# facebookresearch/Pearl

Hardware: NVIDIA H100
Metric: learner gradient-steps/sec (batch=256, 1e6 replay) (higher is better)
Workload: dtype f32 (3xTF32 tensor-core products, fp32 accumulate)

## Files before the change

### pearl_b200/csrc/dqn_common.cuh

```cuda
#pragma once
#include "common.cuh"
#include "host_runtime.cuh"

namespace prl {

struct Dims {
    int obs, A, H1, H2, D, H1p, H2p, P, Pp;
    int oW1, ob1, oW2, ob2, oW3, ob3;
};

__host__ __device__ inline Dims make_dims(int obs, int A, int H1, int H2) {
    Dims d;
    d.obs = obs; d.A = A; d.H1 = H1; d.H2 = H2; d.D = obs + A;
    d.H1p = round_up(H1, 4); d.H2p = round_up(H2, 4);
    d.oW1 = 0; d.ob1 = d.oW1 + H1 * d.D; d.oW2 = d.ob1 + H1; d.ob2 = d.oW2 + H2 * H1;
    d.oW3 = d.ob2 + H2; d.ob3 = d.oW3 + H2; d.P = d.ob3 + 1;
    d.Pp = round_up(d.P + 1, 4);
    return d;
}


__device__ __forceinline__ float soft_update(float src, float tgt, float tau, float omtau) {
    return __fadd_rn(__fmul_rn(tau, src), __fmul_rn(omtau, tgt));
}


struct AdamScalars {
    float decay, omb1, beta2, omb2, eps, step_size, bc2_sqrt;
};
__device__ __forceinline__ float adamw_step(float *w, float *m_, float *v_, float *vmax_, float g, const AdamScalars &h) {
    float p = __fmul_rn(__ldcg(w), h.decay);
    float m = __ldcg(m_);
    m = fmaf(h.omb1, g - m, m);
    float v = __fmul_rn(__ldcg(v_), h.beta2);
    v = __fadd_rn(v, __fmul_rn(__fmul_rn(h.omb2, g), g));
    const float vm = fmaxf(__ldcg(vmax_), v);
    const float denom = __fadd_rn(__fdiv_rn(__fsqrt_rn(vm), h.bc2_sqrt), h.eps);
    p = __fadd_rn(p, __fdiv_rn(__fmul_rn(-h.step_size, m), denom));
    *w = p; *m_ = m; *v_ = v; *vmax_ = vm;
    return p;
}

}

struct prl_dqn {
    prl_dqn_cfg cfg;
    prl::Dims d;
    float *w, *wt, *m, *v, *vmax;
    int64_t adam_step;
    float *gpart;
    int32_t *slots, *logical;
    float2 *scal_dev;
    uint32_t *tmp_rec;
    float *is_w, *td;
    void *multi_dev;
    float *tc_tiles;
    int32_t *tmp_slots;
    prl_buf_layout tmp_lay;
    prl::Stage stage;
    int sm_count, max_smem;
    int learn_smem, qv_smem;
    int last_launches, last_ctas, last_rows;
    int timing;
    cudaEvent_t t0, t1;
    long long *prof;
    prl_comm *comm;
};


int prl_dqn_stage_scalars(prl_dqn *q, int rounds, cudaStream_t stream);

inline int64_t prl_tc_tile_floats(const prl_dqn_cfg *c) {
    if (c->hidden1 != 64 || c->hidden2 != 64 || c->obs_dim > 128 || c->obs_dim % 8) return 0;
    return 2ll * (128 * ((c->obs_dim + 63) & ~63) + 2 * 64 * 64);
}
```

### pearl_b200/csrc/dqn_tc.cu

```cuda
#include <math.h>
#include <stdarg.h>
#include <stdlib.h>

#include <new>

#include "dqn_common.cuh"
#include "sampler.cuh"
#include "umma.cuh"

using namespace prl;

int prl_sampler_params(const prl_buf *b, int k, prl::SamplerParams *sp, size_t *smem_bytes);

namespace {

constexpr int NTH = 256;
constexpr int HID = 64;
constexpr int MAX_B = 256;
constexpr int REG1 = 0, REG2 = 65536, REG3 = 131072, MISC_OFF = 196608;
constexpr int HALF = 32768;
constexpr int SBUF = 16384;
constexpr int TL = 144;
constexpr int AR_A_HI = 0, AR_A_LO = 18432, AR_B_HI = 36864, AR_B_LO = 73728, AR_E = 110592;
constexpr int ACH = 1024, ARING = 8, ASLOT = 4 * ACH * 4;

struct TcLearner {
    const uint32_t *records;
    float *tiles;
    const int32_t *slots;
    float *w, *wt, *m, *v, *vmax;
    const float2 *scal;
    float *out_mae, *out_q, *out_y;
    long long steps0;
    int buf_flags;
    int pad_;
};

struct TcArgs {
    const TcLearner *learners;
    prl_buf_layout lay;
    Dims d;
    int B, rounds, freq;
    int round0;
    float decay, omb1, beta2, omb2, eps, gamma, tau, omtau, inv_b2;
    long long *prof;
    int prof_cta;
    int adam_tma;
};

#define TC_STAMP(idx)                                                                          \
    do {                                                                                       \
        if (a.prof && blockIdx.x == a.prof_cta && threadIdx.x == 0) a.prof[(size_t)round * 16 + (idx)] = clock64(); \
    } while (0)

struct Misc {
    struct Smalls { float watb[16][HID]; float b2[HID], w3[HID]; float b3, pad0[3]; } sm[2];
    float y[MAX_B];
    int act[MAX_B], cnt[MAX_B], slot[MAX_B];
    float rew[MAX_B], term[MAX_B];
    float redw[8][HID];
    float redmae[8], reddb3[8];
    unsigned long long bar[3 + ARING];
    TcLearner L;
    float dw3[16][NTH];
};

__device__ __forceinline__ void cp_async16_zfill_tc(void *smem_dst, const void *gmem_src, int src_bytes) {
    unsigned sa = (unsigned)__cvta_generic_to_shared(smem_dst);
    asm volatile("cp.async.cg.shared.global [%0], [%1], 16, %2;\n" ::"r"(sa), "l"(gmem_src), "r"(src_bytes) : "memory");
}

__device__ __forceinline__ int tid_here() {
    int t = threadIdx.x;
    asm volatile("" : "+r"(t));
    return t;
}
__device__ __forceinline__ int acc_row_here(int p) {
    const int t = tid_here();
    return ((t >> 5) & 3) * 16 + ((t & 31) >> 2) + 8 * p;
}
__device__ __forceinline__ void group_sync(int g) { asm volatile("bar.sync %0, %1;" ::"r"(1 + g), "r"(128) : "memory"); }

__device__ __forceinline__ void mbar_expect_tx(uint64_t *bar, uint32_t bytes) {
    asm volatile("mbarrier.arrive.expect_tx.shared::cta.b64 _, [%0], %1;" ::"r"(umma::smem_u32(bar)), "r"(bytes) : "memory");
}
__device__ __forceinline__ void bulk_g2s(void *smem_dst, const void *gmem_src, uint32_t bytes, uint64_t *bar) {
    asm volatile("cp.async.bulk.shared::cluster.global.mbarrier::complete_tx::bytes [%0], [%1], %2, [%3];"
                 ::"r"(umma::smem_u32(smem_dst)), "l"(gmem_src), "r"(bytes), "r"(umma::smem_u32(bar))
                 : "memory");
}
__device__ __forceinline__ void fence_proxy_async_all() { asm volatile("fence.proxy.async;" ::: "memory"); }
using umma::tf32_lo;

struct NetTiles { float *w1hi, *w1lo, *w2; };
__host__ __device__ inline int k1_cols(int obs) { return (obs + 63) & ~63; }
__host__ __device__ inline int net_tile_floats(int obs) { return 128 * k1_cols(obs) + 2 * HID * HID; }
__device__ __forceinline__ NetTiles net_tiles(float *base, int obs) {
    const int k1 = k1_cols(obs);
    return NetTiles{base, base + 64 * k1, base + 128 * k1};
}
__device__ void rebuild_tiles(const float *__restrict__ net, const Dims &d, const NetTiles &t, int tid) {
    const int k1 = k1_cols(d.obs);
    for (int e = tid; e < HID * k1; e += NTH) {
        const int j = e / k1, k = e - j * k1;
        const float x = k < d.obs ? __ldcg(net + d.oW1 + (size_t)j * d.D + k) : 0.f;
        const int idx = umma::tile_index(j, k, k1);
        t.w1hi[idx] = x; t.w1lo[idx] = tf32_lo(x);
    }
    for (int e = tid; e < HID * HID; e += NTH) {
        const int j = e >> 6, k = e & 63;
        const float x = __ldcg(net + d.oW2 + e);
        const int i1 = umma::tile_index(j, umma::kperm(k), HID);
        t.w2[i1] = x; t.w2[4096 + i1] = tf32_lo(x);
    }
}
__device__ void load_smalls(const float *__restrict__ net, const Dims &d, Misc::Smalls &mi) {
    const int tid = tid_here();
    float wa[4], bb[4];
#pragma unroll
    for (int u = 0; u < 4; u++) {
        const int e = tid + u * NTH;
        if (e < d.A * HID) {
            const int j = e / d.A, a = e - j * d.A;
            wa[u] = __ldcg(net + d.oW1 + (size_t)j * d.D + d.obs + a);
            bb[u] = __ldcg(net + d.ob1 + j);
        }
    }
#pragma unroll
    for (int u = 0; u < 4; u++) {
        const int e = tid + u * NTH;
        if (e < d.A * HID) { const int j = e / d.A, a = e - j * d.A; mi.watb[a][j] = wa[u] + bb[u]; }
    }
    if (tid < HID) { mi.b2[tid] = __ldcg(net + d.ob2 + tid); mi.w3[tid] = __ldcg(net + d.oW3 + tid); }
    if (tid == 0) mi.b3 = __ldcg(net + d.ob3);
}

__device__ __forceinline__ float fast_sqrt(float x) {
    float r;
    asm("sqrt.approx.f32 %0, %1;" : "=f"(r) : "f"(x));
    return r;
}
struct AdamScalarsTc : AdamScalars { float inv_bc2_sqrt; };

__device__ __forceinline__ float adam_math(float w, float &m, float &v, float &x, float g, const AdamScalarsTc &hs) {
    float p = __fmul_rn(w, hs.decay);
    m = fmaf(hs.omb1, g - m, m);
    v = __fadd_rn(__fmul_rn(v, hs.beta2), __fmul_rn(__fmul_rn(hs.omb2, g), g));
    x = fmaxf(x, v);
    const float denom = __fadd_rn(__fmul_rn(fast_sqrt(x), hs.inv_bc2_sqrt), hs.eps);
    return __fadd_rn(p, __fdividef(__fmul_rn(-hs.step_size, m), denom));
}

__device__ __forceinline__ void l1_issue(const TcArgs &a, const TcLearner &L, const Misc &mi, char *smem, int field_off, int row0, int kc) {
    const int ft = tid_here(), m = ft & 127, g = ft >> 7;
    float *sbuf = reinterpret_cast<float *>(smem + REG2 + g * 2 * SBUF + (kc & 1) * SBUF);
#pragma unroll 4
    for (int i = 0; i < 8; i++) {
        const int item = i * 128 + m, rr = item >> 4, c = item & 15, k = kc * 64 + c * 4;
        const float *src = reinterpret_cast<const float *>(L.records + (size_t)mi.slot[row0 + rr] * a.lay.record_words) + field_off + k;
        const int nb = k < a.d.obs ? 16 : 0;
        cp_async16_zfill_tc(sbuf + rr * 64 + ((c ^ (rr & 7)) << 2), nb ? src : reinterpret_cast<const float *>(L.records), nb);
    }
    cp_async_commit();
}
__device__ __forceinline__ void layer1_block(const TcArgs &a, const TcLearner &L, const Misc &mi, char *smem, int field_off, int row0,
                                             float (&t1)[32]) {
// ... 33 lines not shown
            for (int e = 0; e < 2; e++) umma::split_tf32(v[4 * j + 2 * p + e], hi[4 * j + 2 * e + p], lo[4 * j + 2 * e + p]);
}

__device__ __forceinline__ float2 lds2(const float *p) {
    float2 v;
    asm volatile("ld.shared.v2.f32 {%0, %1}, [%2];" : "=f"(v.x), "=f"(v.y) : "r"(umma::smem_u32(p)));
    return v;
}

__device__ __forceinline__ float warp_sum(float v) {
#pragma unroll
    for (int o = 16; o; o >>= 1) v += __shfl_xor_sync(0xffffffffu, v, o);
    return v;
}
__device__ __forceinline__ float quad_sum(float v) {
    v += __shfl_xor_sync(0xffffffffu, v, 1);
    return v + __shfl_xor_sync(0xffffffffu, v, 2);
}

__host__ __device__ inline int dw1_share(int obs) { return obs > 64 ? 64 : obs > 32 ? 32 : obs > 16 ? 16 : 8; }

__device__ const uint8_t kIota[16] = {0, 1, 2, 3, 4, 5, 6, 7, 8, 9, 10, 11, 12, 13, 14, 15};

template <int NW>
__global__ void __launch_bounds__(NTH, 1) k_dqn_tc(const TcArgs a) {
    extern __shared__ __align__(1024) char smem[];
    Misc &mi = *reinterpret_cast<Misc *>(smem + MISC_OFF);
    const int tid = threadIdx.x, warp = tid >> 5, lane = tid & 31;
    if (tid == 0) {
        TcLearner L = a.learners[blockIdx.x];
        if (a.round0) {
            L.slots += (size_t)a.round0 * a.B;
            L.scal += a.round0;
            L.out_mae += a.round0;
            if (L.out_q) L.out_q += (size_t)a.round0 * a.B;
            if (L.out_y) L.out_y += (size_t)a.round0 * a.B;
            L.steps0 += a.round0;
        }
        mi.L = L;
    }
    __syncthreads();
    const TcLearner &L = mi.L;
    const Dims &d = a.d;
    const int h = tid >> 7, t4 = tid & 3;
    const int ntiles = a.B >> 7;
    const int W = a.lay.record_words;

    if (tid == 0 && gridDim.x > 1) {
        const long long t0 = clock64(), wait = (long long)(blockIdx.x % 48) * 2000;
        while (clock64() - t0 < wait) __nanosleep(100);
    }
    uint64_t *bar = reinterpret_cast<uint64_t *>(mi.bar);
    if (tid == 0)
        for (int i = 0; i < 3 + ARING; i++) umma::mbar_init(bar + i, 1);
    auto To = [&] { return net_tiles(L.tiles, d.obs); };
    auto Tt = [&] { return net_tiles(L.tiles + net_tile_floats(d.obs), d.obs); };
    rebuild_tiles(L.w, d, To(), tid);
    rebuild_tiles(L.wt, d, Tt(), tid);
    fence_proxy_async_all();
    __syncthreads();
    const int k1 = k1_cols(d.obs);
    const uint32_t w1_bytes = 64u * k1 * 4, w2_bytes = 2u * HID * HID * 4;
    auto tma_w1 = [&](const NetTiles &t, uint64_t *b) {
        mbar_expect_tx(b, 2 * w1_bytes);
        bulk_g2s(smem + REG1, t.w1hi, w1_bytes, b);
        bulk_g2s(smem + REG1 + HALF, t.w1lo, w1_bytes, b);
    };
    auto tma_w2 = [&](const NetTiles &t, uint64_t *b) {
        mbar_expect_tx(b, w2_bytes);
        bulk_g2s(smem + REG3, t.w2, w2_bytes, b);
    };
    const int an = d.ob2, nch = (an + ACH - 1) / ACH;
    auto aslot = [&](int s) { return smem + (s < 4 ? REG3 : REG1) + (s & 3) * ASLOT; };
    auto adam_issue = [&](int k) {
        const int off = k * ACH, s = k % ARING;
        const uint32_t bytes = 4u * (an - off < ACH ? an - off : ACH);
        char *dst = aslot(s);
        mbar_expect_tx(bar + 3 + s, 4 * bytes);
        bulk_g2s(dst, L.w + off, bytes, bar + 3 + s);
        bulk_g2s(dst + ACH * 4, L.m + off, bytes, bar + 3 + s);
        bulk_g2s(dst + ACH * 8, L.v + off, bytes, bar + 3 + s);
        bulk_g2s(dst + ACH * 12, L.vmax + off, bytes, bar + 3 + s);
    };
    uint32_t par_w1 = 0;
    const umma::Tile W2_hi = umma::make_tile(smem + REG3, 64, 128), W2_lo = umma::make_tile(smem + REG3 + 16384, 64, 128);
    const umma::Tile W2T_hi = umma::make_tile(smem + REG3 + 32768, 64, 128), W2T_lo = umma::make_tile(smem + REG3 + 49152, 64, 128);

    for (int round = 0; round < a.rounds; round++) {
        TC_STAMP(0);
        if (tid < a.B) {
            const int slot = L.slots[(size_t)round * a.B + tid];
            const uint32_t *r = L.records + (size_t)slot * W;
            mi.slot[tid] = slot;
            mi.act[tid] = (int)r[a.lay.off_action];
            mi.rew[tid] = __uint_as_float(r[a.lay.off_reward]);
            const uint32_t fl = r[a.lay.off_flags];
            mi.term[tid] = (fl & 1u) ? 1.f : 0.f;
            mi.cnt[tid] = (int)((fl >> 8) & 0xffffu);
            if (round + 1 < a.rounds) {
                const char *nx = reinterpret_cast<const char *>(L.records + (size_t)L.slots[(size_t)(round + 1) * a.B + tid] * W);
                for (int o = 0; o < W * 4; o += 128) asm volatile("prefetch.global.L2 [%0];" ::"l"(nx + o));
            }
        }
        const bool soft_upd = (L.steps0 + round + 2) % a.freq == 0;
        if (soft_upd) {
            for (int i = tid; i < d.P; i += NTH) L.wt[i] = soft_update(__ldcg(L.w + i), __ldcg(L.wt + i), a.tau, a.omtau);
            auto update_tile = [&](const float *on_hi, float *tg_hi, float *tg_lo, int n) {
                for (int i = tid * 4; i < n; i += NTH * 4) {
                    const float4 w = __ldcg(reinterpret_cast<const float4 *>(on_hi + i)), t = __ldcg(reinterpret_cast<const float4 *>(tg_hi + i));
                    const float4 r = make_float4(soft_update(w.x, t.x, a.tau, a.omtau), soft_update(w.y, t.y, a.tau, a.omtau),
                                                 soft_update(w.z, t.z, a.tau, a.omtau), soft_update(w.w, t.w, a.tau, a.omtau));
                    *reinterpret_cast<float4 *>(tg_hi + i) = r;
                    *reinterpret_cast<float4 *>(tg_lo + i) = make_float4(tf32_lo(r.x), tf32_lo(r.y), tf32_lo(r.z), tf32_lo(r.w));
                }
            };
            update_tile(To().w1hi, Tt().w1hi, Tt().w1lo, HID * k1);
            update_tile(To().w2, Tt().w2, Tt().w2 + HID * HID, HID * HID);
            fence_proxy_async_all();
        }
        __syncthreads();

        TC_STAMP(1);
        if (tid == 0) {
            mbar_expect_tx(bar + 0, 2 * w1_bytes + w2_bytes);
            bulk_g2s(smem + REG1, Tt().w1hi, w1_bytes, bar + 0);
            bulk_g2s(smem + REG1 + HALF, Tt().w1lo, w1_bytes, bar + 0);
            bulk_g2s(smem + REG3, Tt().w2, w2_bytes, bar + 0);
        }
        l1_issue(a, L, mi, smem, a.lay.off_next_state, h * 64, 0);
        if (soft_upd || round == 0) load_smalls(L.wt, d, mi.sm[1]);
        umma::mbar_wait(bar + 0, round & 1);
        __syncthreads();
        TC_STAMP(2);
        for (int i = 0; i < ntiles; i++) {
            const int row0 = i * 128 + h * 64;
// ... 3 lines not shown
            else l1_issue(a, L, mi, smem, a.lay.off_state, h * 64, 0);
            const int rows[2] = {row0 + acc_row_here(0), row0 + acc_row_here(1)};
            int cnt[2];
            const uint8_t *ids[2];
            float best[2] = {-INFINITY, -INFINITY};
#pragma unroll
            for (int p = 0; p < 2; p++) {
                cnt[p] = mi.cnt[rows[p]];
                ids[p] = (L.buf_flags & PRL_BUF_DYNAMIC_ACTIONS) ? reinterpret_cast<const uint8_t *>(L.records + (size_t)mi.slot[rows[p]] * W + a.lay.off_avail)
                                                                : kIota;
            }
            for (int act = 0; act < d.A; act++) {
                const int t4 = tid_here() & 3;
                float hi[32], lo[32], acc[32];
#pragma unroll
                for (int p = 0; p < 2; p++) {
                    const int id_l = ids[p][act], id = act < cnt[p] ? id_l : act;
#pragma unroll
                    for (int j = 0; j < 8; j++) {
                        const float2 wv = lds2(&mi.sm[1].watb[id][8 * j + 2 * t4]);
                        umma::split_tf32(fmaxf(t1[4 * j + 2 * p] + wv.x, 0.f), hi[4 * j + p], lo[4 * j + p]);
                        umma::split_tf32(fmaxf(t1[4 * j + 2 * p + 1] + wv.y, 0.f), hi[4 * j + 2 + p], lo[4 * j + 2 + p]);
                    }
                }
                umma::gemm3_rs<HID, 8>(acc, hi, lo, W2_hi, W2_lo, false);
                umma::wg_commit();
                umma::wg_wait<0>();
                float q[2] = {0.f, 0.f};
#pragma unroll
                for (int j = 0; j < 8; j++) {
                    const float2 w3v = lds2(&mi.sm[1].w3[8 * j + 2 * t4]);
                    const float2 b2v = lds2(&mi.sm[1].b2[8 * j + 2 * t4]);
#pragma unroll
                    for (int p = 0; p < 2; p++) {
                        q[p] = fmaf(w3v.x, fmaxf(acc[4 * j + 2 * p] + b2v.x, 0.f), q[p]);
                        q[p] = fmaf(w3v.y, fmaxf(acc[4 * j + 2 * p + 1] + b2v.y, 0.f), q[p]);
                    }
                }
#pragma unroll
                for (int p = 0; p < 2; p++) {
                    float v = quad_sum(q[p]) + mi.sm[1].b3;
                    if (act >= cnt[p]) v = -INFINITY;
                    best[p] = fmaxf(best[p], v);
                }
            }
            if (t4 == 0)
#pragma unroll
                for (int p = 0; p < 2; p++)
                    mi.y[rows[p]] = __fadd_rn(__fmul_rn(__fmul_rn(best[p], a.gamma), 1.f - mi.term[rows[p]]), mi.rew[rows[p]]);
        }
        __syncthreads();

        TC_STAMP(3);
        if (tid == 0) { tma_w1(To(), bar + 1); tma_w2(To(), bar + 2); }
        load_smalls(L.w, d, mi.sm[0]);
        umma::mbar_wait(bar + 2, round & 1);
        {
            const float *w2 = reinterpret_cast<const float *>(smem + REG3);
            float *w2t = reinterpret_cast<float *>(smem + REG3 + 32768);
            for (int e = tid; e < HID * HID; e += NTH) {
                const int j = e >> 6, k = e & 63, i1 = umma::tile_index(j, umma::kperm(k), HID), i2 = umma::tile_index(k, umma::kperm(j), HID);
                w2t[i2] = w2[i1]; w2t[4096 + i2] = w2[4096 + i1];
            }
            umma::fence_async_smem();
        }
        TC_STAMP(4);
        float gw2[16], gb2[4], gw1[NW / 2], gba[8];
        float mae_acc = 0.f, db3_acc = 0.f;
        float *arena = reinterpret_cast<float *>(smem);
        const umma::Tile TA_hi = umma::make_tile(smem + AR_A_HI, 64, TL), TA_lo = umma::make_tile(smem + AR_A_LO, 64, TL);
        const umma::Tile TB_hi = umma::make_tile(smem + AR_B_HI, 64, TL), TB_lo = umma::make_tile(smem + AR_B_LO, 64, TL);
        const umma::Tile TE = umma::make_tile(smem + AR_E, 64, TL);
        for (int i = 0; i < ntiles; i++) {
            const int row0 = i * 128 + h * 64;
            if (i > 0) {
                if (tid == 0) tma_w1(To(), bar + 1);
                l1_issue(a, L, mi, smem, a.lay.off_state, row0, 0);
            }
            umma::mbar_wait(bar + 1, par_w1);
            par_w1 ^= 1;
            __syncthreads();
            const int rows[2] = {row0 + acc_row_here(0), row0 + acc_row_here(1)};
            float h1[32], z[32], hi[32], lo[32];
            layer1_block(a, L, mi, smem, a.lay.off_state, row0, h1);
            if (i == 0) TC_STAMP(5);
            int ai[2];
#pragma unroll
            for (int p = 0; p < 2; p++) {
                ai[p] = mi.act[rows[p]];
#pragma unroll
                for (int j = 0; j < 8; j++) {
                    const float2 wv = lds2(&mi.sm[0].watb[ai[p]][8 * j + 2 * t4]);
                    h1[4 * j + 2 * p] = fmaxf(h1[4 * j + 2 * p] + wv.x, 0.f);
                    h1[4 * j + 2 * p + 1] = fmaxf(h1[4 * j + 2 * p + 1] + wv.y, 0.f);
                }
            }
            float *h1s = reinterpret_cast<float *>(smem + REG2 + h * 2 * SBUF) + (tid & 127);
#pragma unroll
            for (int c = 0; c < 32; c++) h1s[c * 128] = h1[c];
            acc_to_frag(h1, hi, lo);
            umma::gemm3_rs<HID, 8>(z, hi, lo, W2_hi, W2_lo, false);
            umma::wg_commit();
            umma::wg_wait<0>();
            float part[2] = {0.f, 0.f}, dq[2];
#pragma unroll
            for (int j = 0; j < 8; j++) {
                const float2 w3v = lds2(&mi.sm[0].w3[8 * j + 2 * t4]);
                const float2 b2v = lds2(&mi.sm[0].b2[8 * j + 2 * t4]);
#pragma unroll
                for (int p = 0; p < 2; p++) {
                    z[4 * j + 2 * p] = fmaxf(z[4 * j + 2 * p] + b2v.x, 0.f);
                    z[4 * j + 2 * p + 1] = fmaxf(z[4 * j + 2 * p + 1] + b2v.y, 0.f);
                    part[p] = fmaf(w3v.x, z[4 * j + 2 * p], part[p]);
                    part[p] = fmaf(w3v.y, z[4 * j + 2 * p + 1], part[p]);
                }
            }
#pragma unroll
            for (int p = 0; p < 2; p++) {
                const float q = quad_sum(part[p]) + mi.sm[0].b3;
                const float y = mi.y[rows[p]];
                dq[p] = (q - y) * a.inv_b2;
                if (t4 == 0) {
                    if (L.out_q) L.out_q[(size_t)round * a.B + rows[p]] = q;
                    if (L.out_y) L.out_y[(size_t)round * a.B + rows[p]] = y;
                    mae_acc += fabsf(q - y);
                    db3_acc += dq[p];
                }
            }
#pragma unroll
            for (int j = 0; j < 8; j++) {
                const float2 w3v = lds2(&mi.sm[0].w3[8 * j + 2 * t4]);
                mi.dw3[2 * j][tid] = (i == 0 ? 0.f : mi.dw3[2 * j][tid]) + (dq[0] * z[4 * j] + dq[1] * z[4 * j + 2]);
                mi.dw3[2 * j + 1][tid] = (i == 0 ? 0.f : mi.dw3[2 * j + 1][tid]) + (dq[0] * z[4 * j + 1] + dq[1] * z[4 * j + 3]);
#pragma unroll
                for (int p = 0; p < 2; p++) {
                    z[4 * j + 2 * p] = z[4 * j + 2 * p] > 0.f ? dq[p] * w3v.x : 0.f;
                    z[4 * j + 2 * p + 1] = z[4 * j + 2 * p + 1] > 0.f ? dq[p] * w3v.y : 0.f;
                }
            }
            float dz1[32];
#pragma unroll
            for (int c = 0; c < 32; c++) h1s[(32 + c) * 128] = z[c];
            acc_to_frag(z, hi, lo);
            umma::gemm3_rs<HID, 8>(dz1, hi, lo, W2T_hi, W2T_lo, false);
            umma::wg_commit();
            umma::wg_wait<0>();
#pragma unroll
            for (int c = 0; c < 32; c++) {
                h1[c] = h1s[c * 128];
                z[c] = h1s[(32 + c) * 128];
                dz1[c] = (h1[c] > 0.f) ? dz1[c] : 0.f;
            }
            if (i == 0) TC_STAMP(6);

            for (int hf = 0; hf < 2; hf++) {
                const int ft = tid_here(), h = ft >> 7, t4 = ft & 3, lane = ft & 31, warp = ft >> 5, rA = acc_row_here(0), rB = rA + 8;
                const bool mine = h == hf;
                const bool first = (i == 0 && hf == 0);
                __syncthreads();
                if (mine) {
#pragma unroll
                    for (int j = 0; j < 8; j++)
#pragma unroll
                        for (int p = 0; p < 2; p++)
#pragma unroll
                            for (int e = 0; e < 2; e++) {
                                const int idx = umma::tile_index2(8 * j + 2 * t4 + e, p ? rB : rA, 64, TL), c = 4 * j + 2 * p + e;
                                arena[AR_A_HI / 4 + idx] = z[c]; arena[AR_A_LO / 4 + idx] = tf32_lo(z[c]);
                                arena[AR_B_HI / 4 + idx] = h1[c]; arena[AR_B_LO / 4 + idx] = tf32_lo(h1[c]);
                            }
                } else {
#pragma unroll
                    for (int p = 0; p < 2; p++) {
                        const int r = p ? rB : rA, act = mi.act[i * 128 + hf * 64 + r];
#pragma unroll
                        for (int x = 0; x < 8; x++) {
                            const int er = t4 * 8 + x;
                            arena[AR_E / 4 + umma::tile_index2(er, r, 64, TL)] = (er == 0 || er == act + 1) ? 1.f : 0.f;
                        }
                    }
                }
                umma::fence_async_smem();
                __syncthreads();
                umma::gemm3<32>(gw2, TA_hi, TA_lo, TB_hi.rows_from(32 * h), TB_lo.rows_from(32 * h), 64, !first);
                umma::gemm3<8>(gb2, TA_hi, TA_lo, TE, TE, 64, !first, false, true);
                umma::wg_commit();
                float sv[4][4];
                auto st_rows_load = [&](int r0) {
#pragma unroll
                    for (int ri = 0; ri < 4; ri++) {
                        const int rq = warp + 8 * (r0 + ri);
                        const float *src = reinterpret_cast<const float *>(L.records + (size_t)mi.slot[i * 128 + hf * 64 + rq] * W) + a.lay.off_state;
#pragma unroll
                        for (int jj = 0; jj < 4; jj++) sv[ri][jj] = (lane + 32 * jj < d.obs) ? __ldg(src + lane + 32 * jj) : 0.f;
                    }
                };
                auto st_rows_scatter = [&](int r0) {
#pragma unroll
                    for (int ri = 0; ri < 4; ri++) {
                        const int rq = warp + 8 * (r0 + ri);
#pragma unroll
                        for (int jj = 0; jj < 4; jj++)
                            if (lane + 32 * jj < d.obs) {
                                const int idx = umma::tile_index2(lane + 32 * jj, rq, 64, TL);
                                arena[AR_B_HI / 4 + idx] = sv[ri][jj]; arena[AR_B_LO / 4 + idx] = tf32_lo(sv[ri][jj]);
                            }
                    }
                };
                if (lane < 16 && 32 * (lane & 3) < d.obs) {
                    const float *src = reinterpret_cast<const float *>(L.records + (size_t)mi.slot[i * 128 + hf * 64 + warp + 8 * (lane >> 2)] * W) +
                                       a.lay.off_state + 32 * (lane & 3);
                    asm volatile("prefetch.global.L1 [%0];" ::"l"(src));
                }
                umma::wg_wait<0>();
                __syncthreads();
                st_rows_load(0);
                if (mine) {
#pragma unroll
                    for (int j = 0; j < 8; j++)
#pragma unroll
                        for (int p = 0; p < 2; p++)
#pragma unroll
                            for (int e = 0; e < 2; e++) {
                                const int idx = umma::tile_index2(8 * j + 2 * t4 + e, p ? rB : rA, 64, TL), c = 4 * j + 2 * p + e;
                                arena[AR_A_HI / 4 + idx] = dz1[c]; arena[AR_A_LO / 4 + idx] = tf32_lo(dz1[c]);
                            }
                }
                st_rows_scatter(0);
                st_rows_load(4);
                st_rows_scatter(4);
                umma::fence_async_smem();
                __syncthreads();
                umma::gemm3<NW>(gw1, TA_hi, TA_lo, TB_hi.rows_from(NW * h), TB_lo.rows_from(NW * h), 64, !first);
                umma::gemm3<16>(gba, TA_hi, TA_lo, TE.rows_from(16 * h), TE.rows_from(16 * h), 64, !first, false, true);
                umma::wg_commit();
                umma::wg_wait<0>();
            }
            umma::fence_async_smem();
            __syncthreads();
        }
        if (a.adam_tma && tid == 0)
            for (int k = 0; k < ARING && k < nch; k++) adam_issue(k);

        TC_STAMP(8);
#pragma unroll
        for (int c = 0; c < 16; c++) {
            float v = mi.dw3[c][tid];
            v += __shfl_xor_sync(0xffffffffu, v, 4);
            v += __shfl_xor_sync(0xffffffffu, v, 8);
            v += __shfl_xor_sync(0xffffffffu, v, 16);
            if (lane < 4) mi.redw[warp][8 * (c >> 1) + 2 * lane + (c & 1)] = v;
        }
        {
            const float ms = warp_sum(mae_acc), ds = warp_sum(db3_acc);
            if (lane == 0) { mi.redmae[warp] = ms; mi.reddb3[warp] = ds; }
        }
        {
            float *gs_w2 = reinterpret_cast<float *>(smem + REG2);
            const int pitch1 = d.D | 1;
            float *gs_w1 = gs_w2 + 64 * 65;
            float *gs_b1 = gs_w1 + 64 * pitch1, *gs_b2 = gs_b1 + 64;
#pragma unroll
            for (int p = 0; p < 2; p++) {
                const int j = acc_row_here(p);
#pragma unroll
                for (int jb = 0; jb < 4; jb++)
#pragma unroll
                    for (int e = 0; e < 2; e++) {
                        const int c = 8 * jb + 2 * t4 + e, x = 4 * jb + 2 * p + e;
                        gs_w2[j * 65 + 32 * h + c] = gw2[x];
                        if (jb < NW / 8 && NW * h + c < d.obs) gs_w1[j * pitch1 + NW * h + c] = gw1[x];
                        if (jb < 2) {
                            const int ce = 16 * h + c;
                            if (ce == 0) gs_b1[j] = gba[x];
                            else if (ce - 1 < d.A) gs_w1[j * pitch1 + d.obs + ce - 1] = gba[x];
                        }
                    }
#pragma unroll
                for (int jb = 4; jb < NW / 8; jb++)
#pragma unroll
                    for (int e = 0; e < 2; e++) {
                        const int k = NW * h + 8 * jb + 2 * t4 + e;
                        if (k < d.obs) gs_w1[j * pitch1 + k] = gw1[4 * jb + 2 * p + e];
                    }
                if (h == 0 && t4 == 0) gs_b2[j] = gb2[2 * p];
            }
            __syncthreads();
            TC_STAMP(7);
            const float2 sc = L.scal[round];
            AdamScalarsTc hs;
            hs.decay = a.decay; hs.omb1 = a.omb1; hs.beta2 = a.beta2; hs.omb2 = a.omb2; hs.eps = a.eps;
            hs.step_size = sc.x; hs.bc2_sqrt = sc.y; hs.inv_bc2_sqrt = 1.0f / sc.y;
            int si = -1;
            float sg = 0.f, sw = 0.f, sm = 0.f, sv2 = 0.f, sx = 0.f;
            if (tid < 64) { si = d.ob1 + tid; sg = gs_b1[tid]; }
            else if (tid < 128) { si = d.ob2 + tid - 64; sg = gs_b2[tid - 64]; }
            else if (tid < 192) {
                const int col = tid - 128;
                sg = 0.f;
#pragma unroll
                for (int w8 = 0; w8 < 8; w8++) sg += mi.redw[w8][col];
                si = d.oW3 + col;
            } else if (tid == 192) {
                float e = 0.f;
#pragma unroll
                for (int w8 = 0; w8 < 8; w8++) { sg += mi.reddb3[w8]; e += mi.redmae[w8]; }
                si = d.ob3;
                L.out_mae[round] = e / (float)a.B;
            }
            if (si >= 0) { sw = __ldcg(L.w + si); sm = __ldcg(L.m + si); sv2 = __ldcg(L.v + si); sx = __ldcg(L.vmax + si); }
            if (a.adam_tma) {
                const int n1 = HID * d.D;
                for (int k = 0; k < nch; k++) {
                    const int s = k % ARING, uses = (nch - 1 - s) / ARING + 1;
                    umma::mbar_wait(bar + 3 + s, (uint32_t)(round * uses + k / ARING) & 1u);
                    const int i = k * ACH + 4 * tid;
                    if (i < an && (i < n1 || i >= d.oW2)) {
                        const float4 *sl = reinterpret_cast<const float4 *>(aslot(s)) + tid;
                        float4 w = sl[0], mm = sl[ACH / 4], vv = sl[ACH / 2], xx = sl[3 * ACH / 4];
                        const bool is_w1 = i < n1;
                        int row, c;
                        const float *gp;
                        if (is_w1) {
                            row = i / d.D; c = i - row * d.D;
                            gp = gs_w1 + row * pitch1 + c;
                        } else {
                            const int e = i - d.oW2;
                            row = e >> 6; c = e & 63;
                            gp = gs_w2 + row * 65 + c;
                        }
                        w.x = adam_math(w.x, mm.x, vv.x, xx.x, gp[0], hs); w.y = adam_math(w.y, mm.y, vv.y, xx.y, gp[1], hs);
                        w.z = adam_math(w.z, mm.z, vv.z, xx.z, gp[2], hs); w.w = adam_math(w.w, mm.w, vv.w, xx.w, gp[3], hs);
                        *reinterpret_cast<float4 *>(L.w + i) = w; *reinterpret_cast<float4 *>(L.m + i) = mm;
                        *reinterpret_cast<float4 *>(L.v + i) = vv; *reinterpret_cast<float4 *>(L.vmax + i) = xx;
                        if (is_w1) {
                            if (c < d.obs) {
                                const int ti = umma::tile_index(row, c, k1);
                                *reinterpret_cast<float4 *>(To().w1hi + ti) = w;
                                *reinterpret_cast<float4 *>(To().w1lo + ti) = make_float4(tf32_lo(w.x), tf32_lo(w.y), tf32_lo(w.z), tf32_lo(w.w));
                            }
                        } else {
                            const int te = umma::tile_index(row, umma::kperm(c), HID), to = umma::tile_index(row, umma::kperm(c + 1), HID);
                            *reinterpret_cast<float2 *>(To().w2 + te) = make_float2(w.x, w.z);
                            *reinterpret_cast<float2 *>(To().w2 + to) = make_float2(w.y, w.w);
                            *reinterpret_cast<float2 *>(To().w2 + 4096 + te) = make_float2(tf32_lo(w.x), tf32_lo(w.z));
                            *reinterpret_cast<float2 *>(To().w2 + 4096 + to) = make_float2(tf32_lo(w.y), tf32_lo(w.w));
                        }
                    }
                    if (k + ARING < nch) {
                        __syncthreads();
                        if (tid == 0) adam_issue(k + ARING);
                    }
                }
            } else {
                for (int row = warp; row < HID; row += 8)
                    for (int c = lane; c < d.D; c += 32) {
                        const int i = d.oW1 + row * d.D + c;
                        float mm = __ldcg(L.m + i), vv = __ldcg(L.v + i), xx = __ldcg(L.vmax + i);
                        L.w[i] = adam_math(__ldcg(L.w + i), mm, vv, xx, gs_w1[row * pitch1 + c], hs);
                        L.m[i] = mm; L.v[i] = vv; L.vmax[i] = xx;
                    }
                for (int e = tid; e < HID * HID; e += NTH) {
                    const int i = d.oW2 + e;
                    float mm = __ldcg(L.m + i), vv = __ldcg(L.v + i), xx = __ldcg(L.vmax + i);
                    L.w[i] = adam_math(__ldcg(L.w + i), mm, vv, xx, gs_w2[(e >> 6) * 65 + (e & 63)], hs);
                    L.m[i] = mm; L.v[i] = vv; L.vmax[i] = xx;
                }
                __syncthreads();
                rebuild_tiles(L.w, d, To(), tid);
            }
            TC_STAMP(10);
            fence_proxy_async_all();
            if (si >= 0) {
                L.w[si] = adam_math(sw, sm, sv2, sx, sg, hs);
                L.m[si] = sm; L.v[si] = sv2; L.vmax[si] = sx;
            }
        }
        __syncthreads();
        TC_STAMP(9);
    }
}

__global__ void k_delay(unsigned ns) {
    const long long t0 = clock64();
    while (clock64() - t0 < (long long)ns * 2) __nanosleep(200);
}

struct MultiSampler {
    uint32_t *mt_state;
    SamplerParams sp;
};
__global__ void __launch_bounds__(kSamplerThreads, 1) k_sample_indices_multi(const MultiSampler *items, int rounds, int round0) {
    extern __shared__ __align__(16) unsigned char dyn[];
    __shared__ SamplerState S;
    MultiSampler it = items[blockIdx.x];
    if (it.sp.out_slot) it.sp.out_slot += (size_t)round0 * it.sp.k;
    if (it.sp.out_logical) it.sp.out_logical += (size_t)round0 * it.sp.k;
    sampler_init(S, it.mt_state, dyn, it.sp);
    sampler_advance(S, dyn, it.sp, rounds);
// ... 152 lines not shown
```

### pearl_b200/csrc/umma.cuh

```cuda
#pragma once
#include <cuda_runtime.h>
#include <stdint.h>
#include <stdio.h>

namespace umma {

__device__ __forceinline__ uint32_t smem_u32(const void *p) { return (uint32_t)__cvta_generic_to_shared(p); }

constexpr int LBO = 128;
__host__ __device__ constexpr int tile_sbo(int K) { return (K / 4) * 128; }
__host__ __device__ constexpr int tile_bytes(int rows, int K) { return (rows / 8) * tile_sbo(K); }
__device__ __forceinline__ int tile_index(int r, int k, int K) {
    return (r >> 3) * (tile_sbo(K) >> 2) + (k >> 2) * 32 + (r & 7) * 4 + (k & 3);
}

__device__ __forceinline__ float tf32_lo(float x) { return x - __uint_as_float(__float_as_uint(x) & 0xffffe000u); }
__device__ __forceinline__ void split_tf32(float x, float &hi, float &lo) {
    hi = x;
    lo = tf32_lo(x);
}

__device__ __forceinline__ uint64_t make_desc2(uint32_t smem_addr, int lbo_bytes, int sbo_bytes) {
    uint64_t d = 0;
    d |= (uint64_t)((smem_addr >> 4) & 0x3fff);
// ... 42 lines not shown
                         "wgmma.mma_async.sync.aligned.m64n" #N "k8.f32.tf32.tf32 " DREGS ", %" #A0 ", %" #B0 ", p, 1, 1;\n\t}\n" \
                         : DOPS                                                                                         \
                         : "l"(a_desc), "l"(b_desc), "r"((uint32_t)accumulate));                                        \
        }                                                                                                               \
    };
UMMA_DEFINE(8, "{%0, %1, %2, %3}", UMMA_D4(0), 4, 5, 6)
UMMA_DEFINE(16, "{%0, %1, %2, %3, %4, %5, %6, %7}", UMMA_D8(0), 8, 9, 10)
UMMA_DEFINE(32, "{%0, %1, %2, %3, %4, %5, %6, %7, %8, %9, %10, %11, %12, %13, %14, %15}", UMMA_D16(0), 16, 17, 18)
UMMA_DEFINE(64,
            "{%0, %1, %2, %3, %4, %5, %6, %7, %8, %9, %10, %11, %12, %13, %14, %15, %16, %17, %18, %19, %20, %21, %22, %23, "
            "%24, %25, %26, %27, %28, %29, %30, %31}",
            UMMA_D32(0), 32, 33, 34)
#undef UMMA_DEFINE

template <int N>
__device__ __forceinline__ void mma_rs(float *d, const float *a, uint64_t b_desc, bool accumulate);
template <>
__device__ __forceinline__ void mma_rs<32>(float *d, const float *a, uint64_t b_desc, bool accumulate) {
    asm volatile("{\n\t.reg .pred p;\n\tsetp.ne.b32 p, %21, 0;\n\t"
                 "wgmma.mma_async.sync.aligned.m64n32k8.f32.tf32.tf32 "
                 "{%0, %1, %2, %3, %4, %5, %6, %7, %8, %9, %10, %11, %12, %13, %14, %15}, {%16, %17, %18, %19}, %20, p, 1, 1;\n\t}\n"
                 : UMMA_D16(0)
                 : "r"(__float_as_uint(a[0])), "r"(__float_as_uint(a[1])), "r"(__float_as_uint(a[2])), "r"(__float_as_uint(a[3])),
                   "l"(b_desc), "r"((uint32_t)accumulate));
}
template <>
__device__ __forceinline__ void mma_rs<64>(float *d, const float *a, uint64_t b_desc, bool accumulate) {
    asm volatile("{\n\t.reg .pred p;\n\tsetp.ne.b32 p, %37, 0;\n\t"
                 "wgmma.mma_async.sync.aligned.m64n64k8.f32.tf32.tf32 "
                 "{%0, %1, %2, %3, %4, %5, %6, %7, %8, %9, %10, %11, %12, %13, %14, %15, %16, %17, %18, %19, %20, %21, %22, %23, "
                 "%24, %25, %26, %27, %28, %29, %30, %31}, {%32, %33, %34, %35}, %36, p, 1, 1;\n\t}\n"
                 : UMMA_D32(0)
                 : "r"(__float_as_uint(a[0])), "r"(__float_as_uint(a[1])), "r"(__float_as_uint(a[2])), "r"(__float_as_uint(a[3])),
                   "l"(b_desc), "r"((uint32_t)accumulate));
}
#undef UMMA_D32
#undef UMMA_D16
#undef UMMA_D8
#undef UMMA_D4

template <int N>
__device__ __forceinline__ void gemm3(float *d, Tile a_hi, Tile a_lo, Tile b_hi, Tile b_lo, int K, bool accumulate_first,
                                      bool a_exact = false, bool b_exact = false) {
    bool acc = accumulate_first;
    wg_fence();
    for (int ks = 0; ks < (K >> 3); ks++) {
        if (!a_exact) { Mma<N>::ss(d, a_lo.desc(ks), b_hi.desc(ks), acc); acc = true; }
        if (!b_exact) { Mma<N>::ss(d, a_hi.desc(ks), b_lo.desc(ks), acc); acc = true; }
        Mma<N>::ss(d, a_hi.desc(ks), b_hi.desc(ks), acc);
        acc = true;
    }
}

template <int N, int KSTEPS>
__device__ __forceinline__ void gemm3_rs(float *d, const float *a_hi, const float *a_lo, Tile b_hi, Tile b_lo, bool accumulate_first,
                                         int ksteps = KSTEPS) {
    wg_fence();
#pragma unroll
    for (int ks = 0; ks < KSTEPS; ks++) {
        if (ks >= ksteps) break;
        mma_rs<N>(d, a_lo + 4 * ks, b_hi.desc(ks), accumulate_first || ks > 0);
        mma_rs<N>(d, a_hi + 4 * ks, b_lo.desc(ks), true);
        mma_rs<N>(d, a_hi + 4 * ks, b_hi.desc(ks), true);
    }
}

__device__ __forceinline__ void mbar_init(uint64_t *bar, uint32_t count) {
    asm volatile("mbarrier.init.shared::cta.b64 [%0], %1;" ::"r"(smem_u32(bar)), "r"(count) : "memory");
    asm volatile("fence.mbarrier_init.release.cluster;" ::: "memory");
}
__device__ __forceinline__ void mbar_wait(uint64_t *bar, uint32_t parity) {
    const uint32_t a = smem_u32(bar);
    uint32_t done;
    long long t0 = 0;
    do {
        asm volatile(
            "{\n\t.reg .pred p;\n\t"
            "mbarrier.try_wait.parity.shared::cta.b64 p, [%1], %2;\n\t"
            "selp.b32 %0, 1, 0, p;\n\t}\n"
            : "=r"(done)
            : "r"(a), "r"(parity)
            : "memory");
        if (!done) {
            if (t0 == 0) t0 = clock64();
            if (clock64() - t0 < 3000000000ll) continue;
            __trap();
        }
    } while (!done);
}

}
```

Measured before the change: 511,000.

## Precompute transposed W2 tiles in global and restructure backward gemm phases

Keeps a transposed W2 tile copy in global memory, updated alongside the W2 tiles during the Adam update, and loads it with the same TMA barrier as W1, so the per-round in-shared-memory transpose and its separate barrier go away. The backward pass is split into two loops: the W2-gradient gemms first, then the W1-gradient gemms. When NW is 64, the W1-gradient gemm reads state fragments from registers (gemm3_rs) rather than a scattered shared tile. The shared-memory arena is relaid out and dz1 and h1 are staged in different regions, which adds __syncthreads calls. Profiling stamps become predicated inline asm.

```diff
diff --git a/pearl_b200/csrc/dqn_common.cuh b/pearl_b200/csrc/dqn_common.cuh
--- a/pearl_b200/csrc/dqn_common.cuh
+++ b/pearl_b200/csrc/dqn_common.cuh
@@ -72,5 +72,5 @@
 
 inline int64_t prl_tc_tile_floats(const prl_dqn_cfg *c) {
     if (c->hidden1 != 64 || c->hidden2 != 64 || c->obs_dim > 128 || c->obs_dim % 8) return 0;
-    return 2ll * (128 * ((c->obs_dim + 63) & ~63) + 2 * 64 * 64);
+    return 2ll * (128 * ((c->obs_dim + 63) & ~63) + 2 * 64 * 64) + 2 * 64 * 64;
 }
diff --git a/pearl_b200/csrc/dqn_tc.cu b/pearl_b200/csrc/dqn_tc.cu
--- a/pearl_b200/csrc/dqn_tc.cu
+++ b/pearl_b200/csrc/dqn_tc.cu
@@ -21,7 +21,7 @@
 constexpr int HALF = 32768;
 constexpr int SBUF = 16384;
 constexpr int TL = 144;
-constexpr int AR_A_HI = 0, AR_A_LO = 18432, AR_B_HI = 36864, AR_B_LO = 73728, AR_E = 110592;
+constexpr int AR_A_HI = 0, AR_A_LO = 18432, AR_E = 36864, AR_B_LO = 46080, AR_B_HI = REG3 + HALF;
 constexpr int ACH = 1024, ARING = 8, ASLOT = 4 * ACH * 4;
 
 struct TcLearner {
@@ -48,10 +48,13 @@
     int adam_tma;
 };
 
-#define TC_STAMP(idx)                                                                          \
-    do {                                                                                       \
-        if (a.prof && blockIdx.x == a.prof_cta && threadIdx.x == 0) a.prof[(size_t)round * 16 + (idx)] = clock64(); \
-    } while (0)
+__device__ __forceinline__ void tc_stamp(const TcArgs &a, int round, int idx) {
+    long long *p = a.prof + (size_t)round * 16 + idx;
+    const unsigned on = (a.prof != nullptr) & (blockIdx.x == (unsigned)a.prof_cta) & (threadIdx.x == 0);
+    asm volatile("{\n\t.reg .pred q;\n\t.reg .u64 c;\n\tsetp.ne.u32 q, %1, 0;\n\tmov.u64 c, %%clock64;\n\t@q st.global.u64 [%0], c;\n\t}"
+                 ::"l"(p), "r"(on) : "memory");
+}
+#define TC_STAMP(idx) tc_stamp(a, round, (idx))
 
 struct Misc {
     struct Smalls { float watb[16][HID]; float b2[HID], w3[HID]; float b3, pad0[3]; } sm[2];
@@ -60,7 +63,7 @@
     float rew[MAX_B], term[MAX_B];
     float redw[8][HID];
     float redmae[8], reddb3[8];
-    unsigned long long bar[3 + ARING];
+    unsigned long long bar[2 + ARING];
     TcLearner L;
     float dw3[16][NTH];
 };
@@ -92,12 +95,12 @@
 __device__ __forceinline__ void fence_proxy_async_all() { asm volatile("fence.proxy.async;" ::: "memory"); }
 using umma::tf32_lo;
 
-struct NetTiles { float *w1hi, *w1lo, *w2; };
+struct NetTiles { float *w1hi, *w1lo, *w2, *w2t; };
 __host__ __device__ inline int k1_cols(int obs) { return (obs + 63) & ~63; }
 __host__ __device__ inline int net_tile_floats(int obs) { return 128 * k1_cols(obs) + 2 * HID * HID; }
-__device__ __forceinline__ NetTiles net_tiles(float *base, int obs) {
-    const int k1 = k1_cols(obs);
-    return NetTiles{base, base + 64 * k1, base + 128 * k1};
+__device__ __forceinline__ NetTiles net_tiles(float *base, int obs, bool with_w2t) {
+    const int k1 = k1_cols(obs), n = net_tile_floats(obs);
+    return NetTiles{base, base + 64 * k1, base + 128 * k1, with_w2t ? base + n : nullptr};
 }
 __device__ void rebuild_tiles(const float *__restrict__ net, const Dims &d, const NetTiles &t, int tid) {
     const int k1 = k1_cols(d.obs);
@@ -112,6 +115,10 @@
         const float x = __ldcg(net + d.oW2 + e);
         const int i1 = umma::tile_index(j, umma::kperm(k), HID);
         t.w2[i1] = x; t.w2[4096 + i1] = tf32_lo(x);
+        if (t.w2t) {
+            const int i2 = umma::tile_index(k, umma::kperm(j), HID);
+            t.w2t[i2] = x; t.w2t[4096 + i2] = tf32_lo(x);
+        }
     }
 }
 __device__ void load_smalls(const float *__restrict__ net, const Dims &d, Misc::Smalls &mi) {
@@ -251,23 +258,20 @@
     }
     uint64_t *bar = reinterpret_cast<uint64_t *>(mi.bar);
     if (tid == 0)
-        for (int i = 0; i < 3 + ARING; i++) umma::mbar_init(bar + i, 1);
-    auto To = [&] { return net_tiles(L.tiles, d.obs); };
-    auto Tt = [&] { return net_tiles(L.tiles + net_tile_floats(d.obs), d.obs); };
+        for (int i = 0; i < 2 + ARING; i++) umma::mbar_init(bar + i, 1);
+    auto To = [&] { return net_tiles(L.tiles, d.obs, true); };
+    auto Tt = [&] { return net_tiles(L.tiles + net_tile_floats(d.obs) + 2 * HID * HID, d.obs, false); };
     rebuild_tiles(L.w, d, To(), tid);
     rebuild_tiles(L.wt, d, Tt(), tid);
     fence_proxy_async_all();
     __syncthreads();
     const int k1 = k1_cols(d.obs);
     const uint32_t w1_bytes = 64u * k1 * 4, w2_bytes = 2u * HID * HID * 4;
-    auto tma_w1 = [&](const NetTiles &t, uint64_t *b) {
-        mbar_expect_tx(b, 2 * w1_bytes);
+    auto tma_online = [&](const NetTiles &t, uint64_t *b) {
+        mbar_expect_tx(b, 2 * w1_bytes + 2 * w2_bytes);
         bulk_g2s(smem + REG1, t.w1hi, w1_bytes, b);
         bulk_g2s(smem + REG1 + HALF, t.w1lo, w1_bytes, b);
-    };
-    auto tma_w2 = [&](const NetTiles &t, uint64_t *b) {
-        mbar_expect_tx(b, w2_bytes);
-        bulk_g2s(smem + REG3, t.w2, w2_bytes, b);
+        bulk_g2s(smem + REG3, t.w2, 2 * w2_bytes, b);
     };
     const int an = d.ob2, nch = (an + ACH - 1) / ACH;
     auto aslot = [&](int s) { return smem + (s < 4 ? REG3 : REG1) + (s & 3) * ASLOT; };
@@ -275,11 +279,11 @@
         const int off = k * ACH, s = k % ARING;
         const uint32_t bytes = 4u * (an - off < ACH ? an - off : ACH);
         char *dst = aslot(s);
-        mbar_expect_tx(bar + 3 + s, 4 * bytes);
-        bulk_g2s(dst, L.w + off, bytes, bar + 3 + s);
-        bulk_g2s(dst + ACH * 4, L.m + off, bytes, bar + 3 + s);
-        bulk_g2s(dst + ACH * 8, L.v + off, bytes, bar + 3 + s);
-        bulk_g2s(dst + ACH * 12, L.vmax + off, bytes, bar + 3 + s);
+        mbar_expect_tx(bar + 2 + s, 4 * bytes);
+        bulk_g2s(dst, L.w + off, bytes, bar + 2 + s);
+        bulk_g2s(dst + ACH * 4, L.m + off, bytes, bar + 2 + s);
+        bulk_g2s(dst + ACH * 8, L.v + off, bytes, bar + 2 + s);
+        bulk_g2s(dst + ACH * 12, L.vmax + off, bytes, bar + 2 + s);
     };
     uint32_t par_w1 = 0;
     const umma::Tile W2_hi = umma::make_tile(smem + REG3, 64, 128), W2_lo = umma::make_tile(smem + REG3 + 16384, 64, 128);
@@ -389,18 +393,8 @@
         __syncthreads();
 
         TC_STAMP(3);
-        if (tid == 0) { tma_w1(To(), bar + 1); tma_w2(To(), bar + 2); }
+        if (tid == 0) tma_online(To(), bar + 1);
         load_smalls(L.w, d, mi.sm[0]);
-        umma::mbar_wait(bar + 2, round & 1);
-        {
-            const float *w2 = reinterpret_cast<const float *>(smem + REG3);
-            float *w2t = reinterpret_cast<float *>(smem + REG3 + 32768);
-            for (int e = tid; e < HID * HID; e += NTH) {
-                const int j = e >> 6, k = e & 63, i1 = umma::tile_index(j, umma::kperm(k), HID), i2 = umma::tile_index(k, umma::kperm(j), HID);
-                w2t[i2] = w2[i1]; w2t[4096 + i2] = w2[4096 + i1];
-            }
-            umma::fence_async_smem();
-        }
         TC_STAMP(4);
         float gw2[16], gb2[4], gw1[NW / 2], gba[8];
         float mae_acc = 0.f, db3_acc = 0.f;
@@ -408,10 +402,21 @@
         const umma::Tile TA_hi = umma::make_tile(smem + AR_A_HI, 64, TL), TA_lo = umma::make_tile(smem + AR_A_LO, 64, TL);
         const umma::Tile TB_hi = umma::make_tile(smem + AR_B_HI, 64, TL), TB_lo = umma::make_tile(smem + AR_B_LO, 64, TL);
         const umma::Tile TE = umma::make_tile(smem + AR_E, 64, TL);
+        auto e_scatter = [&](int b0, int rA, int rB, int t4) {
+#pragma unroll
+            for (int p = 0; p < 2; p++) {
+                const int r = p ? rB : rA, act = mi.act[b0 + r];
+#pragma unroll
+                for (int x = 0; x < 8; x++) {
+                    const int er = t4 * 8 + x;
+                    arena[AR_E / 4 + umma::tile_index2(er, r, 64, TL)] = (er == 0 || er == act + 1) ? 1.f : 0.f;
+                }
+            }
+        };
         for (int i = 0; i < ntiles; i++) {
             const int row0 = i * 128 + h * 64;
             if (i > 0) {
-                if (tid == 0) tma_w1(To(), bar + 1);
+                if (tid == 0) tma_online(To(), bar + 1);
                 l1_issue(a, L, mi, smem, a.lay.off_state, row0, 0);
             }
             umma::mbar_wait(bar + 1, par_w1);
@@ -420,6 +425,7 @@
             const int rows[2] = {row0 + acc_row_here(0), row0 + acc_row_here(1)};
             float h1[32], z[32], hi[32], lo[32];
             layer1_block(a, L, mi, smem, a.lay.off_state, row0, h1);
+            __syncthreads();
             if (i == 0) TC_STAMP(5);
             int ai[2];
 #pragma unroll
@@ -432,7 +438,7 @@
                     h1[4 * j + 2 * p + 1] = fmaxf(h1[4 * j + 2 * p + 1] + wv.y, 0.f);
                 }
             }
-            float *h1s = reinterpret_cast<float *>(smem + REG2 + h * 2 * SBUF) + (tid & 127);
+            float *h1s = reinterpret_cast<float *>(smem + REG1 + h * HALF) + (tid & 127);
 #pragma unroll
             for (int c = 0; c < 32; c++) h1s[c * 128] = h1[c];
             acc_to_frag(h1, hi, lo);
@@ -488,6 +494,10 @@
                 z[c] = h1s[(32 + c) * 128];
                 dz1[c] = (h1[c] > 0.f) ? dz1[c] : 0.f;
             }
+            __syncthreads();
+            float *dzs = reinterpret_cast<float *>(smem + REG3 + h * (HALF / 2)) + (tid & 127);
+#pragma unroll
+            for (int c = 0; c < 32; c++) dzs[c * 128] = dz1[c];
             if (i == 0) TC_STAMP(6);
 
             for (int hf = 0; hf < 2; hf++) {
@@ -507,21 +517,27 @@
                                 arena[AR_B_HI / 4 + idx] = h1[c]; arena[AR_B_LO / 4 + idx] = tf32_lo(h1[c]);
                             }
                 } else {
-#pragma unroll
-                    for (int p = 0; p < 2; p++) {
-                        const int r = p ? rB : rA, act = mi.act[i * 128 + hf * 64 + r];
-#pragma unroll
-                        for (int x = 0; x < 8; x++) {
-                            const int er = t4 * 8 + x;
-                            arena[AR_E / 4 + umma::tile_index2(er, r, 64, TL)] = (er == 0 || er == act + 1) ? 1.f : 0.f;
-                        }
-                    }
+                    e_scatter(i * 128 + hf * 64, rA, rB, t4);
                 }
                 umma::fence_async_smem();
                 __syncthreads();
+                if (first) TC_STAMP(11);
                 umma::gemm3<32>(gw2, TA_hi, TA_lo, TB_hi.rows_from(32 * h), TB_lo.rows_from(32 * h), 64, !first);
                 umma::gemm3<8>(gb2, TA_hi, TA_lo, TE, TE, 64, !first, false, true);
                 umma::wg_commit();
+                if (NW < 64 && lane < 16 && 32 * (lane & 3) < d.obs) {
+                    const float *src = reinterpret_cast<const float *>(L.records + (size_t)mi.slot[i * 128 + hf * 64 + warp + 8 * (lane >> 2)] * W) +
+                                       a.lay.off_state + 32 * (lane & 3);
+                    asm volatile("prefetch.global.L1 [%0];" ::"l"(src));
+                }
+                umma::wg_wait<0>();
+                if (first) TC_STAMP(12);
+            }
+            for (int hf = 0; hf < 2; hf++) {
+                const int ft = tid_here(), h = ft >> 7, t4 = ft & 3, lane = ft & 31, warp = ft >> 5, rA = acc_row_here(0), rB = rA + 8;
+                const bool mine = h == hf;
+                const bool first = (i == 0 && hf == 0);
+                __syncthreads();
                 float sv[4][4];
                 auto st_rows_load = [&](int r0) {
 #pragma unroll
@@ -544,14 +560,7 @@
                             }
                     }
                 };
-                if (lane < 16 && 32 * (lane & 3) < d.obs) {
-                    const float *src = reinterpret_cast<const float *>(L.records + (size_t)mi.slot[i * 128 + hf * 64 + warp + 8 * (lane >> 2)] * W) +
-                                       a.lay.off_state + 32 * (lane & 3);
-                    asm volatile("prefetch.global.L1 [%0];" ::"l"(src));
-                }
-                umma::wg_wait<0>();
-                __syncthreads();
-                st_rows_load(0);
+                if constexpr (NW < 64) st_rows_load(0);
                 if (mine) {
 #pragma unroll
                     for (int j = 0; j < 8; j++)
@@ -560,18 +569,40 @@
 #pragma unroll
                             for (int e = 0; e < 2; e++) {
                                 const int idx = umma::tile_index2(8 * j + 2 * t4 + e, p ? rB : rA, 64, TL), c = 4 * j + 2 * p + e;
-                                arena[AR_A_HI / 4 + idx] = dz1[c]; arena[AR_A_LO / 4 + idx] = tf32_lo(dz1[c]);
+                                const float v = reinterpret_cast<const float *>(smem + REG3 + h * (HALF / 2))[c * 128 + (ft & 127)];
+                                arena[AR_A_HI / 4 + idx] = v; arena[AR_A_LO / 4 + idx] = tf32_lo(v);
                             }
-                }
-                st_rows_scatter(0);
-                st_rows_load(4);
-                st_rows_scatter(4);
+                } else {
+                    e_scatter(i * 128 + hf * 64, rA, rB, t4);
+                }
+                if constexpr (NW < 64) {
+                    st_rows_scatter(0);
+                    st_rows_load(4);
+                    st_rows_scatter(4);
+                }
                 umma::fence_async_smem();
                 __syncthreads();
-                umma::gemm3<NW>(gw1, TA_hi, TA_lo, TB_hi.rows_from(NW * h), TB_lo.rows_from(NW * h), 64, !first);
+                if (first) TC_STAMP(13);
+                if constexpr (NW == 64) {
+                    const float *sbuf = reinterpret_cast<const float *>(smem + REG2 + hf * 2 * SBUF + h * SBUF);
+                    float shi[32], slo[32];
+#pragma unroll
+                    for (int ks = 0; ks < 8; ks++)
+#pragma unroll
+                        for (int q = 0; q < 2; q++)
+#pragma unroll
+                            for (int p = 0; p < 2; p++) {
+                                const int o = p ? rB : rA, r = 8 * ks + t4 + 4 * q;
+                                umma::split_tf32(sbuf[r * 64 + (((o >> 2) ^ (r & 7)) << 2) + (o & 3)], shi[4 * ks + 2 * q + p], slo[4 * ks + 2 * q + p]);
+                            }
+                    umma::gemm3_rs<64, 8, true>(gw1, shi, slo, TA_hi, TA_lo, !first);
+                } else {
+                    umma::gemm3<NW>(gw1, TA_hi, TA_lo, TB_hi.rows_from(NW * h), TB_lo.rows_from(NW * h), 64, !first);
+                }
                 umma::gemm3<16>(gba, TA_hi, TA_lo, TE.rows_from(16 * h), TE.rows_from(16 * h), 64, !first, false, true);
                 umma::wg_commit();
                 umma::wg_wait<0>();
+                if (first) TC_STAMP(14);
             }
             umma::fence_async_smem();
             __syncthreads();
@@ -606,20 +637,21 @@
                     for (int e = 0; e < 2; e++) {
                         const int c = 8 * jb + 2 * t4 + e, x = 4 * jb + 2 * p + e;
                         gs_w2[j * 65 + 32 * h + c] = gw2[x];
-                        if (jb < NW / 8 && NW * h + c < d.obs) gs_w1[j * pitch1 + NW * h + c] = gw1[x];
+                        if (NW < 64 && jb < NW / 8 && NW * h + c < d.obs) gs_w1[j * pitch1 + NW * h + c] = gw1[x];
                         if (jb < 2) {
                             const int ce = 16 * h + c;
                             if (ce == 0) gs_b1[j] = gba[x];
                             else if (ce - 1 < d.A) gs_w1[j * pitch1 + d.obs + ce - 1] = gba[x];
                         }
                     }
-#pragma unroll
-                for (int jb = 4; jb < NW / 8; jb++)
-#pragma unroll
-                    for (int e = 0; e < 2; e++) {
-                        const int k = NW * h + 8 * jb + 2 * t4 + e;
-                        if (k < d.obs) gs_w1[j * pitch1 + k] = gw1[4 * jb + 2 * p + e];
-                    }
+                if constexpr (NW == 64) {
+                    const int k = 64 * h + j;
+#pragma unroll
+                    for (int jb = 0; jb < 8; jb++)
+#pragma unroll
+                        for (int e = 0; e < 2; e++)
+                            if (k < d.obs) gs_w1[(8 * jb + 2 * t4 + e) * pitch1 + k] = gw1[4 * jb + 2 * p + e];
+                }
                 if (h == 0 && t4 == 0) gs_b2[j] = gb2[2 * p];
             }
             __syncthreads();
@@ -650,7 +682,7 @@
                 const int n1 = HID * d.D;
                 for (int k = 0; k < nch; k++) {
                     const int s = k % ARING, uses = (nch - 1 - s) / ARING + 1;
-                    umma::mbar_wait(bar + 3 + s, (uint32_t)(round * uses + k / ARING) & 1u);
+                    umma::mbar_wait(bar + 2 + s, (uint32_t)(round * uses + k / ARING) & 1u);
                     const int i = k * ACH + 4 * tid;
                     if (i < an && (i < n1 || i >= d.oW2)) {
                         const float4 *sl = reinterpret_cast<const float4 *>(aslot(s)) + tid;
@@ -682,6 +714,14 @@
                             *reinterpret_cast<float2 *>(To().w2 + to) = make_float2(w.y, w.w);
                             *reinterpret_cast<float2 *>(To().w2 + 4096 + te) = make_float2(tf32_lo(w.x), tf32_lo(w.z));
                             *reinterpret_cast<float2 *>(To().w2 + 4096 + to) = make_float2(tf32_lo(w.y), tf32_lo(w.w));
+                            float *w2t = To().w2t;
+                            const int kr = umma::kperm(row);
+                            const float wv[4] = {w.x, w.y, w.z, w.w};
+#pragma unroll
+                            for (int u = 0; u < 4; u++) {
+                                const int ti = umma::tile_index(c + u, kr, HID);
+                                w2t[ti] = wv[u]; w2t[4096 + ti] = tf32_lo(wv[u]);
+                            }
                         }
                     }
                     if (k + ARING < nch) {
diff --git a/pearl_b200/csrc/umma.cuh b/pearl_b200/csrc/umma.cuh
--- a/pearl_b200/csrc/umma.cuh
+++ b/pearl_b200/csrc/umma.cuh
@@ -118,15 +118,20 @@
     }
 }
 
-template <int N, int KSTEPS>
+template <int N, int KSTEPS, bool B_LO_FIRST = false>
 __device__ __forceinline__ void gemm3_rs(float *d, const float *a_hi, const float *a_lo, Tile b_hi, Tile b_lo, bool accumulate_first,
                                          int ksteps = KSTEPS) {
     wg_fence();
 #pragma unroll
     for (int ks = 0; ks < KSTEPS; ks++) {
         if (ks >= ksteps) break;
-        mma_rs<N>(d, a_lo + 4 * ks, b_hi.desc(ks), accumulate_first || ks > 0);
-        mma_rs<N>(d, a_hi + 4 * ks, b_lo.desc(ks), true);
+        if (B_LO_FIRST) {
+            mma_rs<N>(d, a_hi + 4 * ks, b_lo.desc(ks), accumulate_first || ks > 0);
+            mma_rs<N>(d, a_lo + 4 * ks, b_hi.desc(ks), true);
+        } else {
+            mma_rs<N>(d, a_lo + 4 * ks, b_hi.desc(ks), accumulate_first || ks > 0);
+            mma_rs<N>(d, a_hi + 4 * ks, b_lo.desc(ks), true);
+        }
         mma_rs<N>(d, a_hi + 4 * ks, b_hi.desc(ks), true);
     }
 }
```

After: 546,000, median of 6. +6.9%, better.
